# multimodallearning/DG-TTA

Measured on AMD Instinct MI355X. Metric: TTA-epochs/sec per GPU on 128^3 patch; Dice delta vs reference, higher is better.
Workload: dtype fp16

## Files before the change

### dg_tta_amd/_lib.py

```python
import ctypes as C
import os
from pathlib import Path

LIB_PATH = Path(__file__).resolve().parent / "libdgtta_hip.so"

_c_float_p = C.POINTER(C.c_float)
P, I, I64, F, SZ = C.c_void_p, C.c_int, C.c_int64, C.c_float, C.c_size_t

SIGNATURES = {
    "dgtta_version": (I, []),
    "dgtta_last_error": (C.c_char_p, []),
    "dgtta_reload_env": (I, []),
    "dgtta_mind3d_ws_bytes": (SZ, [I, I, I, I]),
    "dgtta_mind3d_fwd": (I, [P, P, F, I, C.POINTER(F), I, P, I, I, I, P, SZ, I, I, I, I, P]),
    "dgtta_gin_ws_bytes": (SZ, [I, I, I, I]),
    "dgtta_gin_chain_fwd": (I, [P, P, C.POINTER(I), C.POINTER(P), C.POINTER(P), P, P, SZ, I, I, I, I, P]),
    "dgtta_affine_warp3d_fwd": (I, [P, P, P, I, I, I, I, I, I, I, I, I, I, I, I, I, I, P, P]),
    "dgtta_affine_warp3d_bwd": (I, [P, P, P, I, I, I, I, I, I, I, I, I, I, I, I, I, P]),
    "dgtta_rf_field_ws_bytes": (SZ, [I, I, I, I]),
    "dgtta_rf_field_fwd": (I, [P, P, P, SZ, I, I, I, I, I, I, I, I, P]),
    "dgtta_diffeo_fields_ws_bytes": (SZ, [I, I, I, I]),
    "dgtta_diffeo_fields": (I, [P, F, P, P, P, SZ, I, I, I, I, I, P]),
    "dgtta_dense_warp3d_fwd": (I, [P, P, P, I, I, I, I, I, I, I, I, I, P]),
    "dgtta_dense_warp3d_bwd": (I, [P, P, P, I, I, I, I, I, I, I, I, I, P]),
    "dgtta_softdice_ws_bytes": (SZ, [I, I, I64]),
    "dgtta_softdice_fwd": (I, [P, P, P, P, P, SZ, I, I, I64, I, I, I, P]),
    "dgtta_softdice_bwd": (I, [P, P, P, P, P, F, P, I, I, I64, I, I, P]),
    "dgtta_softdice_bwd_t": (I, [P, P, P, P, P, F, P, I, I, I64, I, I, I, P]),
    "dgtta_softdice_probs_fwd": (I, [P, P, P, P, SZ, I, I, I64, I64, I64, I64, P]),
    "dgtta_softdice_probs_bwd": (I, [P, P, P, P, P, P, I, I, I64, I64, I64, I64, P]),
    "dgtta_dice_ce_ws_bytes": (SZ, [I, I, I64]),
    "dgtta_dice_ce_fwd": (I, [P, I, P, P, P, P, SZ, I, I, I64, F, I, P]),
    "dgtta_dice_ce_bwd": (I, [P, I, P, P, F, P, P, I, I, I, I64, P]),
    "dgtta_adamw_step": (I, [C.POINTER(P), C.POINTER(P), C.POINTER(P), C.POINTER(P), C.POINTER(I64), I, F, F, F, F, F,
                             I, F, P, P]),
    "dgtta_grads_nonfinite": (I, [C.POINTER(P), C.POINTER(I64), I, P, P]),
    "dgtta_conv3d_packed_bytes": (SZ, [I, I, I]),
    "dgtta_conv3d_pack_weights": (I, [P, P, I, I, I, I, I, P]),
    "dgtta_conv3d_stats_bytes": (SZ, [I, I, I, I, I]),
# ... 106 lines not shown
```

### dg_tta_amd/csrc/gin.hip

```cpp
#include "common.h"

namespace {

constexpr int TD = 8, TH = 8, TW = 32, HALO = 4, NT = 512;
constexpr int R0D = TD + 8, R0H = TH + 8, R0W = TW + 8;
constexpr int PW0 = 40, PW1 = 36, PW2 = 36, PW3 = 32;
constexpr int SZ_A = 2 * (TD + 4) * (TH + 4) * PW1 + 8;
constexpr int SZ_B = 2 * (TD + 6) * (TH + 6) * PW0 + 8;
constexpr int WTAB = 336;

struct GinArgs {
  const float *ker[4];
  const float *shift[4];
  int ksz[4];
};

__device__ __forceinline__ bool inside(int d, int h, int w, int D, int H, int W) {
  return (unsigned)d < (unsigned)D && (unsigned)h < (unsigned)H && (unsigned)w < (unsigned)W;
}

__global__ void gin_prep_kernel(GinArgs a, float *__restrict__ wtab) {
  const int b = blockIdx.x, tid = threadIdx.x;
  const int cin[4] = {1, 2, 2, 2}, cout[4] = {2, 2, 2, 1}, off[4] = {0, 54, 162, 270};
  float *wt = wtab + (int64_t)b * WTAB;
  for (int l = 0; l < 4; ++l) {
    const int k = a.ksz[l], rows = cout[l] * cin[l];
    for (int i = tid; i < rows * 27; i += blockDim.x) {
      const int r = i / 27, t = i % 27, co = r / cin[l], ci = r % cin[l];
      const float v = (k == 3) ? a.ker[l][((int64_t)b * rows + r) * 27 + t]
                               : ((t == 13) ? a.ker[l][(int64_t)b * rows + r] : 0.f);
      wt[off[l] + (ci * 27 + t) * cout[l] + co] = v;
    }
    if (tid < cout[l]) wt[324 + 2 * l + tid] = a.shift[l][b * cout[l] + tid];
  }
}

typedef __attribute__((ext_vector_type(2))) float f32x2_t;

__device__ __forceinline__ void pk_fma_blo(f32x2_t &acc, const f32x2_t &w, const f32x2_t &v) {
  asm volatile("v_pk_fma_f32 %0, %1, %2, %0 op_sel_hi:[1,0,1]" : "+v"(acc) : "v"(w), "v"(v));
}
__device__ __forceinline__ void pk_fma_bhi(f32x2_t &acc, const f32x2_t &w, const f32x2_t &v) {
  asm volatile("v_pk_fma_f32 %0, %1, %2, %0 op_sel:[0,1,0]" : "+v"(acc) : "v"(w), "v"(v));
}

template <int CIN, int COUT, bool ACT, int OD, int OH, int OW, int IPW, int OPW>
__device__ __forceinline__ void gin_layer(const float *sin, float *sout, const float *__restrict__ w ,
                                          const float *__restrict__ sh, int gd0, int gh0, int gw0, int D, int H, int W) {
  constexpr int ID = OD + 2, IH = OH + 2, NSX = (OW + 3) / 4, N = OD * OH * NSX;
  f32x2_t wreg[COUT == 2 ? CIN * 27 : 1];
  if (COUT == 2) {
#pragma unroll
    for (int i = 0; i < CIN * 27; ++i) wreg[i] = f32x2_t{w[2 * i], w[2 * i + 1]};
  }
  for (int s = threadIdx.x; s < N; s += NT) {
    const int xs = (s % NSX) * 4, y = (s / NSX) % OH, z = s / (NSX * OH);
    float o[COUT][4];
    if (COUT == 2) {
      f32x2_t acc[4];
#pragma unroll
      for (int j = 0; j < 4; ++j) acc[j] = f32x2_t{0.f, 0.f};
#pragma unroll
      for (int ci = 0; ci < CIN; ++ci)
#pragma unroll
        for (int kd = 0; kd < 3; ++kd)
#pragma unroll
          for (int kh = 0; kh < 3; ++kh) {
            const float *p = sin + ((ci * ID + z + kd) * IH + y + kh) * IPW + xs;
            const float4 q0 = *reinterpret_cast<const float4 *>(p);
            const float2 q1 = *reinterpret_cast<const float2 *>(p + 4);
            const f32x2_t vp[3] = {f32x2_t{q0.x, q0.y}, f32x2_t{q0.z, q0.w}, f32x2_t{q1.x, q1.y}};
#pragma unroll
            for (int kw = 0; kw < 3; ++kw) {
              const f32x2_t wv = wreg[ci * 27 + kd * 9 + kh * 3 + kw];
#pragma unroll
              for (int j = 0; j < 4; ++j) {
                if ((j + kw) & 1) pk_fma_bhi(acc[j], wv, vp[(j + kw) >> 1]);
                else pk_fma_blo(acc[j], wv, vp[(j + kw) >> 1]);
              }
            }
          }
#pragma unroll
      for (int j = 0; j < 4; ++j) {
        o[0][j] = acc[j][0];
        o[COUT - 1][j] = acc[j][1];
      }
    } else {
      float acc[4] = {0.f, 0.f, 0.f, 0.f};
#pragma unroll
      for (int ci = 0; ci < CIN; ++ci)
#pragma unroll
        for (int kd = 0; kd < 3; ++kd)
#pragma unroll
          for (int kh = 0; kh < 3; ++kh) {
            const float *p = sin + ((ci * ID + z + kd) * IH + y + kh) * IPW + xs;
            const float4 q0 = *reinterpret_cast<const float4 *>(p);
            const float2 q1 = *reinterpret_cast<const float2 *>(p + 4);
            const float v[6] = {q0.x, q0.y, q0.z, q0.w, q1.x, q1.y};
#pragma unroll
            for (int kw = 0; kw < 3; ++kw) {
              const float wv = w[ci * 27 + kd * 9 + kh * 3 + kw];
#pragma unroll
              for (int j = 0; j < 4; ++j) acc[j] = __builtin_fmaf(wv, v[j + kw], acc[j]);
            }
          }
#pragma unroll
      for (int j = 0; j < 4; ++j) o[0][j] = acc[j];
    }
    const bool zy_in = (unsigned)(gd0 + z) < (unsigned)D && (unsigned)(gh0 + y) < (unsigned)H;
#pragma unroll
    for (int co = 0; co < COUT; ++co) {
#pragma unroll
      for (int j = 0; j < 4; ++j) {
        const float v = o[co][j] + sh[co];
        const bool in = zy_in && (unsigned)(gw0 + xs + j) < (unsigned)W;
        o[co][j] = in ? (ACT ? lrelu(v, 0.01f) : v) : 0.f;
      }
      *reinterpret_cast<float4 *>(sout + ((co * OD + z) * OH + y) * OPW + xs) =
          make_float4(o[co][0], o[co][1], o[co][2], o[co][3]);
    }
  }
}

template <int CIN, int COUT, bool ACT, int OD, int OH, int OW, int IPW, int OPW>
__device__ __forceinline__ void gin_layer_k1(const float *sin, float *sout, const float *__restrict__ w,
                                             const float *__restrict__ sh, int gd0, int gh0, int gw0, int D, int H, int W) {
  constexpr int ID = OD + 2, IH = OH + 2, NSX = (OW + 3) / 4, N = OD * OH * NSX;
  float wc[COUT][CIN];
#pragma unroll
  for (int co = 0; co < COUT; ++co)
#pragma unroll
    for (int ci = 0; ci < CIN; ++ci) wc[co][ci] = w[(ci * 27 + 13) * COUT + co];
  for (int s = threadIdx.x; s < N; s += NT) {
    const int xs = (s % NSX) * 4, y = (s / NSX) % OH, z = s / (NSX * OH);
    float v[CIN][4];
#pragma unroll
    for (int ci = 0; ci < CIN; ++ci) {
      const float *p = sin + ((ci * ID + z + 1) * IH + y + 1) * IPW + xs + 1;
#pragma unroll
      for (int j = 0; j < 4; ++j) v[ci][j] = p[j];
    }
    const bool zy_in = (unsigned)(gd0 + z) < (unsigned)D && (unsigned)(gh0 + y) < (unsigned)H;
#pragma unroll
    for (int co = 0; co < COUT; ++co) {
      float o[4];
#pragma unroll
      for (int j = 0; j < 4; ++j) {
        float a = 0.f;
#pragma unroll
        for (int ci = 0; ci < CIN; ++ci) a = __builtin_fmaf(wc[co][ci], v[ci][j], a);
        a += sh[co];
        const bool in = zy_in && (unsigned)(gw0 + xs + j) < (unsigned)W;
        o[j] = in ? (ACT ? lrelu(a, 0.01f) : a) : 0.f;
      }
      *reinterpret_cast<float4 *>(sout + ((co * OD + z) * OH + y) * OPW + xs) = make_float4(o[0], o[1], o[2], o[3]);
    }
  }
}

__global__ __launch_bounds__(NT) void gin_chain_kernel(const float *__restrict__ x, const float *__restrict__ alpha,
                                                       const float *__restrict__ wtab, float *__restrict__ mixed,
                                                       double *__restrict__ partial, int D, int H, int W, int tilesD,
                                                       int tilesH, int tilesW, int ntiles, int k0, int k1, int k2,
                                                       int k3) {
  __shared__ __attribute__((aligned(16))) float bufA[SZ_A];
  __shared__ __attribute__((aligned(16))) float bufB[SZ_B];
  __shared__ float sred[16];
  constexpr int NPRE = R0D * R0H * R0W / NT;
  static_assert(R0D * R0H * R0W % NT == 0, "input tile must divide over the threads");

  const int tid = threadIdx.x;
  const int64_t V = (int64_t)D * H * W;
  const int per = tilesD * tilesH * tilesW;
  float pre[NPRE];
  auto fetch = [&](int tile) {
    const int b = tile / per, bid = tile % per;
    const int d0 = (bid / (tilesH * tilesW)) * TD, h0 = ((bid / tilesW) % tilesH) * TH, w0 = (bid % tilesW) * TW;
    const float *xb = x + (int64_t)b * V;
#pragma unroll
    for (int k = 0; k < NPRE; ++k) {
      const int i = tid + k * NT;
      const int iw = i % R0W, ih = (i / R0W) % R0H, id = i / (R0W * R0H);
      const int gd = d0 - HALO + id, gh = h0 - HALO + ih, gw = w0 - HALO + iw;
      const bool in = inside(gd, gh, gw, D, H, W);
      const float v = xb[in ? ((int64_t)gd * H + gh) * W + gw : 0];
      pre[k] = in ? v : 0.f;
    }
  };
  int tile = blockIdx.x;
  if (tile < ntiles) fetch(tile);
  for (; tile < ntiles; tile += gridDim.x) {
    const int b = tile / per, bid = tile % per;
    const int d0 = (bid / (tilesH * tilesW)) * TD, h0 = ((bid / tilesW) % tilesH) * TH, w0 = (bid % tilesW) * TW;
    const float *xb = x + (int64_t)b * V;
    const float *wt = wtab + (int64_t)b * WTAB;
#pragma unroll
    for (int k = 0; k < NPRE; ++k) bufA[tid + k * NT] = pre[k];
    __syncthreads();
    if (tile + (int)gridDim.x < ntiles) fetch(tile + gridDim.x);
    if (k0 == 1) gin_layer_k1<1, 2, true, TD + 6, TH + 6, TW + 6, R0W, PW0>(bufA, bufB, wt + 0, wt + 324, d0 - 3, h0 - 3, w0 - 3, D, H, W);
    else gin_layer<1, 2, true, TD + 6, TH + 6, TW + 6, R0W, PW0>(bufA, bufB, wt + 0, wt + 324, d0 - 3, h0 - 3, w0 - 3, D, H, W);
    __syncthreads();
    if (k1 == 1) gin_layer_k1<2, 2, true, TD + 4, TH + 4, TW + 4, PW0, PW1>(bufB, bufA, wt + 54, wt + 326, d0 - 2, h0 - 2, w0 - 2, D, H, W);
    else gin_layer<2, 2, true, TD + 4, TH + 4, TW + 4, PW0, PW1>(bufB, bufA, wt + 54, wt + 326, d0 - 2, h0 - 2, w0 - 2, D, H, W);
    __syncthreads();
    if (k2 == 1) gin_layer_k1<2, 2, true, TD + 2, TH + 2, TW + 2, PW1, PW2>(bufA, bufB, wt + 162, wt + 328, d0 - 1, h0 - 1, w0 - 1, D, H, W);
    else gin_layer<2, 2, true, TD + 2, TH + 2, TW + 2, PW1, PW2>(bufA, bufB, wt + 162, wt + 328, d0 - 1, h0 - 1, w0 - 1, D, H, W);
    __syncthreads();
    if (k3 == 1) gin_layer_k1<2, 1, false, TD, TH, TW, PW2, PW3>(bufB, bufA, wt + 270, wt + 330, d0, h0, w0, D, H, W);
    else gin_layer<2, 1, false, TD, TH, TW, PW2, PW3>(bufB, bufA, wt + 270, wt + 330, d0, h0, w0, D, H, W);
    __syncthreads();

    const float al = alpha[b];
    const float om = 1.0f - al;
    float s_in = 0.f, s_mx = 0.f;
    for (int i = tid; i < TD * TH * TW; i += NT) {
      int xw = i % TW, y = (i / TW) % TH, z = i / (TW * TH);
      int gd = d0 + z, gh = h0 + y, gw = w0 + xw;
      if (inside(gd, gh, gw, D, H, W)) {
        int64_t g = ((int64_t)gd * H + gh) * W + gw;
        float xi = xb[g];
        float t1 = al * bufA[i];
        float t2 = om * xi;
        float mx = t1 + t2;
        mixed[(int64_t)b * V + g] = mx;
        s_in += xi * xi;
        s_mx += mx * mx;
      }
    }
    float tin = block_sum(s_in, sred);
    float tmx = block_sum(s_mx, sred);
    if (tid == 0) {
      partial[((int64_t)b * per + bid) * 2 + 0] = (double)tin;
      partial[((int64_t)b * per + bid) * 2 + 1] = (double)tmx;
    }
    __syncthreads();
  }
}

__global__ void gin_norm_kernel(const double *__restrict__ partial, int per, float *__restrict__ norms) {
  __shared__ double sh[2][256];
  const int b = blockIdx.x;
  double s0 = 0.0, s1 = 0.0;
  for (int i = threadIdx.x; i < per; i += 256) {
    s0 += partial[((int64_t)b * per + i) * 2 + 0];
    s1 += partial[((int64_t)b * per + i) * 2 + 1];
  }
  sh[0][threadIdx.x] = s0;
  sh[1][threadIdx.x] = s1;
  __syncthreads();
  for (int o = 128; o > 0; o >>= 1) {
    if ((int)threadIdx.x < o) {
      sh[0][threadIdx.x] += sh[0][threadIdx.x + o];
      sh[1][threadIdx.x] += sh[1][threadIdx.x + o];
    }
    __syncthreads();
  }
  if (threadIdx.x == 0) {
    norms[2 * b + 0] = sqrtf((float)sh[0][0]);
    norms[2 * b + 1] = sqrtf((float)sh[1][0]);
  }
}

__global__ void gin_scale_kernel(float *__restrict__ out, const float *__restrict__ norms, int64_t V, int64_t total) {
  for (int64_t i = (int64_t)blockIdx.x * blockDim.x + threadIdx.x; i < total; i += (int64_t)gridDim.x * blockDim.x) {
    int64_t b = i / V;
    float r = 1.0f / (norms[2 * b + 1] + 1e-5f);
    out[i] = (out[i] * r) * norms[2 * b + 0];
  }
}

}

extern "C" size_t dgtta_gin_ws_bytes(int B, int D, int H, int W) {
  if (B <= 0 || D <= 0 || H <= 0 || W <= 0) return 0;
  size_t per = (size_t)cdiv(D, TD) * cdiv(H, TH) * cdiv(W, TW);
  return align_up((size_t)B * per * 2 * sizeof(double), 256) + align_up((size_t)B * 2 * sizeof(float), 256) +
         align_up((size_t)B * WTAB * sizeof(float), 256);
}

extern "C" int dgtta_gin_chain_fwd(const float *x, const float *alpha, const int *h_ksz, const float *const *h_ker,
                                   const float *const *h_shift, float *out, void *ws, size_t ws_bytes, int B, int D,
                                   int H, int W, void *stream) {
  DG_REQUIRE(x && alpha && h_ksz && h_ker && h_shift && out && ws, DGTTA_ERR_BADARG, "gin_chain_fwd: null pointer");
  DG_REQUIRE(B > 0 && D > 0 && H > 0 && W > 0, DGTTA_ERR_BADARG, "gin_chain_fwd: bad dims");
  DG_REQUIRE(ws_bytes >= dgtta_gin_ws_bytes(B, D, H, W), DGTTA_ERR_WORKSPACE, "gin_chain_fwd: workspace too small");
  GinArgs a;
  for (int l = 0; l < 4; ++l) {
    DG_REQUIRE(h_ksz[l] == 1 || h_ksz[l] == 3, DGTTA_ERR_UNSUPPORTED, "gin_chain_fwd: kernel size %d not in {1,3}",
               h_ksz[l]);
    DG_REQUIRE(h_ker[l] && h_shift[l], DGTTA_ERR_BADARG, "gin_chain_fwd: null layer pointer");
    a.ker[l] = h_ker[l];
    a.shift[l] = h_shift[l];
    a.ksz[l] = h_ksz[l];
  }
  hipStream_t st = (hipStream_t)stream;
  const int td = cdiv(D, TD), th = cdiv(H, TH), tw = cdiv(W, TW);
  DG_REQUIRE((int64_t)td * th * tw * B < (1ll << 31), DGTTA_ERR_UNSUPPORTED, "gin_chain_fwd: volume too large");
  const int per = td * th * tw;
  double *partial = (double *)ws;
  float *norms = (float *)((char *)ws + align_up((size_t)B * per * 2 * sizeof(double), 256));
  float *wtab = (float *)((char *)norms + align_up((size_t)B * 2 * sizeof(float), 256));
  const int64_t V = (int64_t)D * H * W;
  hipLaunchKernelGGL(gin_prep_kernel, dim3(B), dim3(128), 0, st, a, wtab);
  DG_CHECK_LAUNCH("gin_prep_kernel");
  const int ntiles = B * per;
  static const int ncu = [] {
    int dev = 0, n = 256;
    if (hipGetDevice(&dev) == hipSuccess) (void)hipDeviceGetAttribute(&n, hipDeviceAttributeMultiprocessorCount, dev);
    return n > 0 ? n : 256;
  }();
  hipLaunchKernelGGL(gin_chain_kernel, dim3(ntiles < ncu ? ntiles : ncu), dim3(NT), 0, st, x, alpha, wtab, out, partial, D,
                     H, W, td, th, tw, ntiles, a.ksz[0], a.ksz[1], a.ksz[2], a.ksz[3]);
  DG_CHECK_LAUNCH("gin_chain_kernel");
  hipLaunchKernelGGL(gin_norm_kernel, dim3(B), dim3(256), 0, st, partial, per, norms);
  DG_CHECK_LAUNCH("gin_norm_kernel");
  const int64_t total = (int64_t)B * V;
  int blocks = (int)((total + 255) / 256 < 4096 ? (total + 255) / 256 : 4096);
  hipLaunchKernelGGL(gin_scale_kernel, dim3(blocks), dim3(256), 0, st, out, norms, V, total);
  DG_CHECK_LAUNCH("gin_scale_kernel");
  return DGTTA_OK;
}
```

### dg_tta_amd/ops.py

```python
import ctypes as C

import torch

from . import _lib
from ._lib import check, ptr, require_cuda, stream_of

F32, BF16, F16 = 0, 1, 2


def dtype_code(torch_dtype):
    try:
        return {torch.float32: F32, torch.bfloat16: BF16, torch.float16: F16}[torch_dtype]
    except KeyError:
        raise ValueError(f"unsupported activation dtype {torch_dtype}") from None
PAD_ZEROS, PAD_BORDER = 0, 1
LINEAR, NEAREST = 0, 1


def _ws(nbytes, device):
    return torch.empty(max(int(nbytes), 256), dtype=torch.uint8, device=device)


def _f32c(t):
    return t.contiguous().float() if (t.dtype != torch.float32 or not t.is_contiguous()) else t
# ... 38 lines not shown
                                   ptr(out[sl]), int(ndhwc),
                                   int(out_ldc), dtype_code(out_dtype), ptr(ws), nbytes, bg, d, h, w,
                                   stream_of(img.device)), "dgtta_mind3d_fwd")
    return out


def gin_chain(x, alpha, ks, kers, shifts):
    require_cuda(x, alpha, *kers, *shifts)
    lib = _lib.load()
    b, c, d, h, w = x.shape
    assert c == 1 and len(ks) == len(kers) == len(shifts) == 4
    x = _f32c(x)
    alpha = _f32c(alpha)
    kers = [_f32c(k) for k in kers]
    shifts = [_f32c(s) for s in shifts]
    out = torch.empty_like(x)
    nbytes = lib.dgtta_gin_ws_bytes(b, d, h, w)
    ws = _ws(nbytes, x.device)
    ksz = (C.c_int * 4)(*[int(k) for k in ks])
    kp = (C.c_void_p * 4)(*[k.data_ptr() for k in kers])
    sp = (C.c_void_p * 4)(*[s.data_ptr() for s in shifts])
    check(lib.dgtta_gin_chain_fwd(ptr(x), ptr(alpha), ksz, kp, sp, ptr(out), ptr(ws), nbytes, b, d, h, w,
                                  stream_of(x.device)), "dgtta_gin_chain_fwd")
    return out


def _warp_layout(t):
    if is_cl3d(t) and t.shape[1] > 1:
        return t, 1, t.shape[1]
    t = t.contiguous()
    return t, 0, 0


def _warp_fwd_raw(src, theta, out_size, pad_mode, interp, algebra, sub_const):
    lib = _lib.load()
    b, c, ds, hs, wsz = src.shape
    dd, hd, wd = out_size
    src, ndhwc, ldc = _warp_layout(src)
    dst = empty_cl3d(b, c, dd, hd, wd, torch.float32, src.device) if ndhwc else \
        torch.empty((b, c, dd, hd, wd), dtype=torch.float32, device=src.device)
    check(lib.dgtta_affine_warp3d_fwd(ptr(src), ptr(theta), ptr(dst), b, c, ds, hs, wsz, dd, hd, wd, ndhwc, ldc, ldc,
                                      pad_mode, interp, int(algebra), ptr(sub_const), stream_of(src.device)),
          "dgtta_affine_warp3d_fwd")
    return dst


# ... 379 lines not shown
```

### include/dgtta.h

```cpp
#ifndef DGTTA_H
#define DGTTA_H

#include <stddef.h>
#include <stdint.h>

#ifdef __cplusplus
extern "C" {
#endif

#define DGTTA_OK 0
#define DGTTA_ERR_BADARG (-1)
#define DGTTA_ERR_UNSUPPORTED (-2)
#define DGTTA_ERR_WORKSPACE (-3)
#define DGTTA_ERR_LAUNCH (-4)

#define DGTTA_F32 0
#define DGTTA_BF16 1
#define DGTTA_F16 2

#define DGTTA_PAD_ZEROS 0
#define DGTTA_PAD_BORDER 1
#define DGTTA_INTERP_LINEAR 0
#define DGTTA_INTERP_NEAREST 1

int dgtta_version(void);
const char *dgtta_last_error(void);
int dgtta_reload_env(void);

size_t dgtta_mind3d_ws_bytes(int B, int D, int H, int W);
int dgtta_mind3d_fwd(const float *img, const float *noise, float randn_weighting, int delta, const float *h_taps,
                     int ntaps, void *out, int out_ndhwc, int out_ldc, int out_dtype, void *ws, size_t ws_bytes, int B,
                     int D, int H, int W, void *stream);

size_t dgtta_gin_ws_bytes(int B, int D, int H, int W);
int dgtta_gin_chain_fwd(const float *x, const float *alpha, const int *h_ksz, const float *const *h_ker,
                        const float *const *h_shift, float *out, void *ws, size_t ws_bytes, int B, int D, int H,
                        int W, void *stream);

int dgtta_affine_warp3d_fwd(const float *src, const float *theta, float *dst, int B, int C, int Ds, int Hs,
                            int Ws, int Dd, int Hd, int Wd, int ndhwc, int src_ldc, int dst_ldc, int pad_mode,
                            int interp_mode, int tta_grid_algebra, const float *sub_const_dev, void *stream);
int dgtta_affine_warp3d_bwd(const float *grad_dst, const float *theta, float *grad_src, int B, int C, int Ds,
                            int Hs, int Ws, int Dd, int Hd, int Wd, int ndhwc, int src_ldc, int dst_ldc,
                            int pad_mode, int tta_grid_algebra, void *stream);

size_t dgtta_rf_field_ws_bytes(int P, int Dl, int Hl, int Wl);
int dgtta_rf_field_fwd(const float *draw, float *field, void *ws, size_t ws_bytes, int P, int k, int Dl, int Hl, int Wl,
                       int D, int H, int W, void *stream);
size_t dgtta_diffeo_fields_ws_bytes(int N, int D, int H, int W);
int dgtta_diffeo_fields(const float *field, float factor, float *disp, float *inverse, void *ws, size_t ws_bytes, int N,
                        int D, int H, int W, int time_steps, void *stream);
int dgtta_dense_warp3d_fwd(const float *src, const float *disp, float *dst, int B, int C, int D, int H, int W, int ndhwc,
                           int src_ldc, int dst_ldc, int pad_mode, void *stream);
int dgtta_dense_warp3d_bwd(const float *grad_dst, const float *disp, float *grad_src, int B, int C, int D, int H, int W,
                           int ndhwc, int src_ldc, int dst_ldc, int pad_mode, void *stream);

size_t dgtta_softdice_ws_bytes(int B, int C, int64_t V);
int dgtta_softdice_fwd(const float *la, const float *lb, float *dice, float *loss, void *ws, size_t ws_bytes,
                       int B, int C, int64_t V, int ldc, int start_class, int guard_items, void *stream);
int dgtta_softdice_bwd(const float *la, const float *lb, float *grad_la, float *grad_lb, const void *ws,
// ... 164 lines not shown
```

Baseline: 6.529.

## Restructure GIN chain kernel as depth-marching ring-buffered layer pipeline

Replaces the 3D-tile GIN conv chain, which recomputed halos across all four layers in a shared-memory cube, with a kernel that marches along depth over an H×W column. Each layer runs in its own thread role and keeps only a four-plane ring buffer in shared memory, and thread roles stay a fixed number of planes apart, separated by barriers. Weights are held in registers per role, and the depth range is split into segments to fill the CUs. The aim is to cut redundant halo recomputation and shared-memory footprint. It also adds a per-sample GIN weight entry point and batched weight prep. The cost is a larger block, a barrier on every plane step, and more complex partial-sum indexing.

```diff
diff --git a/dg_tta_amd/_lib.py b/dg_tta_amd/_lib.py
--- a/dg_tta_amd/_lib.py
+++ b/dg_tta_amd/_lib.py
@@ -15,6 +15,7 @@
     "dgtta_mind3d_fwd": (I, [P, P, F, I, C.POINTER(F), I, P, I, I, I, P, SZ, I, I, I, I, P]),
     "dgtta_gin_ws_bytes": (SZ, [I, I, I, I]),
     "dgtta_gin_chain_fwd": (I, [P, P, C.POINTER(I), C.POINTER(P), C.POINTER(P), P, P, SZ, I, I, I, I, P]),
+    "dgtta_gin_chain_fwd_per_sample": (I, [P, P, C.POINTER(I), C.POINTER(P), C.POINTER(P), P, P, SZ, I, I, I, I, P]),
     "dgtta_affine_warp3d_fwd": (I, [P, P, P, I, I, I, I, I, I, I, I, I, I, I, I, I, I, P, P]),
     "dgtta_affine_warp3d_bwd": (I, [P, P, P, I, I, I, I, I, I, I, I, I, I, I, I, I, P]),
     "dgtta_rf_field_ws_bytes": (SZ, [I, I, I, I]),
diff --git a/dg_tta_amd/csrc/gin.hip b/dg_tta_amd/csrc/gin.hip
--- a/dg_tta_amd/csrc/gin.hip
+++ b/dg_tta_amd/csrc/gin.hip
@@ -1,37 +1,38 @@
 #include "common.h"
 
+#include <vector>
+
 namespace {
 
-constexpr int TD = 8, TH = 8, TW = 32, HALO = 4, NT = 512;
-constexpr int R0D = TD + 8, R0H = TH + 8, R0W = TW + 8;
-constexpr int PW0 = 40, PW1 = 36, PW2 = 36, PW3 = 32;
-constexpr int SZ_A = 2 * (TD + 4) * (TH + 4) * PW1 + 8;
-constexpr int SZ_B = 2 * (TD + 6) * (TH + 6) * PW0 + 8;
+constexpr int CH = 16, CW = 32, NTM = 768, RING = 4, DBLK = 8;
+constexpr int INH = CH + 8, INPW = 40, IN_SZ = INH * INPW;
+constexpr int H0 = CH + 6, PW0 = 40, SZ0 = 2 * H0 * PW0;
+constexpr int H1 = CH + 4, PW1 = 36, SZ1 = 2 * H1 * PW1;
+constexpr int H2 = CH + 2, PW2 = 36, SZ2 = 2 * H2 * PW2;
 constexpr int WTAB = 336;
 
+constexpr int PREP_B = 8;
 struct GinArgs {
-  const float *ker[4];
-  const float *shift[4];
-  int ksz[4];
+  const float *ker[PREP_B][4];
+  const float *shift[PREP_B][4];
+  int ksz[PREP_B][4];
+  int b0;
 };
 
-__device__ __forceinline__ bool inside(int d, int h, int w, int D, int H, int W) {
-  return (unsigned)d < (unsigned)D && (unsigned)h < (unsigned)H && (unsigned)w < (unsigned)W;
-}
-
 __global__ void gin_prep_kernel(GinArgs a, float *__restrict__ wtab) {
-  const int b = blockIdx.x, tid = threadIdx.x;
+  const int i = blockIdx.x, tid = threadIdx.x;
   const int cin[4] = {1, 2, 2, 2}, cout[4] = {2, 2, 2, 1}, off[4] = {0, 54, 162, 270};
-  float *wt = wtab + (int64_t)b * WTAB;
+  float *wt = wtab + (int64_t)(a.b0 + i) * WTAB;
   for (int l = 0; l < 4; ++l) {
-    const int k = a.ksz[l], rows = cout[l] * cin[l];
-    for (int i = tid; i < rows * 27; i += blockDim.x) {
-      const int r = i / 27, t = i % 27, co = r / cin[l], ci = r % cin[l];
-      const float v = (k == 3) ? a.ker[l][((int64_t)b * rows + r) * 27 + t]
-                               : ((t == 13) ? a.ker[l][(int64_t)b * rows + r] : 0.f);
+    const int k = a.ksz[i][l], rows = cout[l] * cin[l];
+    const float *ker = a.ker[i][l];
+    for (int e = tid; e < rows * 27; e += blockDim.x) {
+      const int r = e / 27, t = e % 27, co = r / cin[l], ci = r % cin[l];
+      const float v = (k == 3) ? ker[r * 27 + t] : ((t == 13) ? ker[r] : 0.f);
       wt[off[l] + (ci * 27 + t) * cout[l] + co] = v;
     }
-    if (tid < cout[l]) wt[324 + 2 * l + tid] = a.shift[l][b * cout[l] + tid];
+    if (tid < cout[l]) wt[324 + 2 * l + tid] = a.shift[i][l][tid];
+    if (tid == 0) wt[332 + l] = (float)k;
   }
 }
 
@@ -44,197 +45,283 @@
   asm volatile("v_pk_fma_f32 %0, %1, %2, %0 op_sel:[0,1,0]" : "+v"(acc) : "v"(w), "v"(v));
 }
 
-template <int CIN, int COUT, bool ACT, int OD, int OH, int OW, int IPW, int OPW>
-__device__ __forceinline__ void gin_layer(const float *sin, float *sout, const float *__restrict__ w ,
-                                          const float *__restrict__ sh, int gd0, int gh0, int gw0, int D, int H, int W) {
-  constexpr int ID = OD + 2, IH = OH + 2, NSX = (OW + 3) / 4, N = OD * OH * NSX;
-  f32x2_t wreg[COUT == 2 ? CIN * 27 : 1];
-  if (COUT == 2) {
-#pragma unroll
-    for (int i = 0; i < CIN * 27; ++i) wreg[i] = f32x2_t{w[2 * i], w[2 * i + 1]};
-  }
-  for (int s = threadIdx.x; s < N; s += NT) {
-    const int xs = (s % NSX) * 4, y = (s / NSX) % OH, z = s / (NSX * OH);
-    float o[COUT][4];
-    if (COUT == 2) {
-      f32x2_t acc[4];
-#pragma unroll
-      for (int j = 0; j < 4; ++j) acc[j] = f32x2_t{0.f, 0.f};
-#pragma unroll
-      for (int ci = 0; ci < CIN; ++ci)
-#pragma unroll
-        for (int kd = 0; kd < 3; ++kd)
-#pragma unroll
-          for (int kh = 0; kh < 3; ++kh) {
-            const float *p = sin + ((ci * ID + z + kd) * IH + y + kh) * IPW + xs;
-            const float4 q0 = *reinterpret_cast<const float4 *>(p);
-            const float2 q1 = *reinterpret_cast<const float2 *>(p + 4);
-            const f32x2_t vp[3] = {f32x2_t{q0.x, q0.y}, f32x2_t{q0.z, q0.w}, f32x2_t{q1.x, q1.y}};
-#pragma unroll
-            for (int kw = 0; kw < 3; ++kw) {
-              const f32x2_t wv = wreg[ci * 27 + kd * 9 + kh * 3 + kw];
-#pragma unroll
-              for (int j = 0; j < 4; ++j) {
-                if ((j + kw) & 1) pk_fma_bhi(acc[j], wv, vp[(j + kw) >> 1]);
-                else pk_fma_blo(acc[j], wv, vp[(j + kw) >> 1]);
-              }
+template <int CIN, int COUT, bool K1>
+struct LayerW {
+  f32x2_t pk[(!K1 && COUT == 2) ? CIN * 27 : 1];
+  float sc[(!K1 && COUT == 1) ? CIN * 27 : 1];
+  float c1[COUT][CIN];
+  float sh[COUT];
+  __device__ __forceinline__ void load(const float *__restrict__ w, const float *__restrict__ shp) {
+    if constexpr (K1) {
+#pragma unroll
+      for (int co = 0; co < COUT; ++co)
+#pragma unroll
+        for (int ci = 0; ci < CIN; ++ci) c1[co][ci] = w[(ci * 27 + 13) * COUT + co];
+    } else if constexpr (COUT == 2) {
+#pragma unroll
+      for (int i = 0; i < CIN * 27; ++i) {
+        pk[i] = f32x2_t{w[2 * i], w[2 * i + 1]};
+        asm volatile("" : "+v"(pk[i]));
+      }
+    } else {
+#pragma unroll
+      for (int i = 0; i < CIN * 27; ++i) sc[i] = w[i];
+    }
+#pragma unroll
+    for (int co = 0; co < COUT; ++co) sh[co] = shp[co];
+  }
+};
+
+template <int CIN, int COUT, bool K1, int IH, int IPW>
+__device__ __forceinline__ void gin_strip(const float *const (&pl)[3], const LayerW<CIN, COUT, K1> &lw, int y, int xs,
+                                          float (&o)[COUT][4]) {
+  if constexpr (K1) {
+    float v[CIN][4];
+#pragma unroll
+    for (int ci = 0; ci < CIN; ++ci) {
+      const float *p = pl[1] + (ci * IH + y + 1) * IPW + xs + 1;
+#pragma unroll
+      for (int j = 0; j < 4; ++j) v[ci][j] = p[j];
+    }
+#pragma unroll
+    for (int co = 0; co < COUT; ++co)
+#pragma unroll
+      for (int j = 0; j < 4; ++j) {
+        float a = 0.f;
+#pragma unroll
+        for (int ci = 0; ci < CIN; ++ci) a = __builtin_fmaf(lw.c1[co][ci], v[ci][j], a);
+        o[co][j] = a;
+      }
+  } else if constexpr (COUT == 2) {
+    f32x2_t acc[4];
+#pragma unroll
+    for (int j = 0; j < 4; ++j) acc[j] = f32x2_t{0.f, 0.f};
+#pragma unroll
+    for (int ci = 0; ci < CIN; ++ci)
+#pragma unroll
+      for (int kd = 0; kd < 3; ++kd)
+#pragma unroll
+        for (int kh = 0; kh < 3; ++kh) {
+          const float *p = pl[kd] + (ci * IH + y + kh) * IPW + xs;
+          const float4 q0 = *reinterpret_cast<const float4 *>(p);
+          const float2 q1 = *reinterpret_cast<const float2 *>(p + 4);
+          const f32x2_t vp[3] = {f32x2_t{q0.x, q0.y}, f32x2_t{q0.z, q0.w}, f32x2_t{q1.x, q1.y}};
+#pragma unroll
+          for (int kw = 0; kw < 3; ++kw) {
+            const f32x2_t wv = lw.pk[ci * 27 + kd * 9 + kh * 3 + kw];
+#pragma unroll
+            for (int j = 0; j < 4; ++j) {
+              if ((j + kw) & 1) pk_fma_bhi(acc[j], wv, vp[(j + kw) >> 1]);
+              else pk_fma_blo(acc[j], wv, vp[(j + kw) >> 1]);
             }
           }
-#pragma unroll
-      for (int j = 0; j < 4; ++j) {
-        o[0][j] = acc[j][0];
-        o[COUT - 1][j] = acc[j][1];
+        }
+#pragma unroll
+    for (int j = 0; j < 4; ++j) {
+      o[0][j] = acc[j][0];
+      o[COUT - 1][j] = acc[j][1];
+    }
+  } else {
+    float acc[4] = {0.f, 0.f, 0.f, 0.f};
+#pragma unroll
+    for (int ci = 0; ci < CIN; ++ci)
+#pragma unroll
+      for (int kd = 0; kd < 3; ++kd)
+#pragma unroll
+        for (int kh = 0; kh < 3; ++kh) {
+          const float *p = pl[kd] + (ci * IH + y + kh) * IPW + xs;
+          const float4 q0 = *reinterpret_cast<const float4 *>(p);
+          const float2 q1 = *reinterpret_cast<const float2 *>(p + 4);
+          const float v[6] = {q0.x, q0.y, q0.z, q0.w, q1.x, q1.y};
+#pragma unroll
+          for (int kw = 0; kw < 3; ++kw) {
+            const float wv = lw.sc[ci * 27 + kd * 9 + kh * 3 + kw];
+#pragma unroll
+            for (int j = 0; j < 4; ++j) acc[j] = __builtin_fmaf(wv, v[j + kw], acc[j]);
+          }
+        }
+#pragma unroll
+    for (int j = 0; j < 4; ++j) o[0][j] = acc[j];
+  }
+}
+
+__device__ __forceinline__ int ring_slot(int p) { return (p + 8) & (RING - 1); }
+
+template <int CIN, bool K1, int IH, int IPW, int ISZ, int OH, int OPW>
+__device__ __forceinline__ void gin_plane_strip(const float *rin, float *po, const LayerW<CIN, 2, K1> &lw, int p, int y,
+                                                int xs, int gh, int gw0, int D, int H, int W) {
+  float o[2][4];
+  const bool row_in = (unsigned)p < (unsigned)D && (unsigned)gh < (unsigned)H;
+  if ((unsigned)p < (unsigned)D) {
+    const float *const pl[3] = {rin + ring_slot(p - 1) * ISZ, rin + ring_slot(p) * ISZ, rin + ring_slot(p + 1) * ISZ};
+    gin_strip<CIN, 2, K1, IH, IPW>(pl, lw, y, xs, o);
+  } else {
+#pragma unroll
+    for (int j = 0; j < 4; ++j) o[0][j] = o[1][j] = 0.f;
+  }
+#pragma unroll
+  for (int co = 0; co < 2; ++co) {
+#pragma unroll
+    for (int j = 0; j < 4; ++j) {
+      const float v = o[co][j] + lw.sh[co];
+      const bool in = row_in && (unsigned)(gw0 + xs + j) < (unsigned)W;
+      o[co][j] = in ? lrelu(v, 0.01f) : 0.f;
+    }
+    *reinterpret_cast<float4 *>(po + (co * OH + y) * OPW + xs) = make_float4(o[co][0], o[co][1], o[co][2], o[co][3]);
+  }
+}
+
+struct March {
+  const float *xb;
+  const float *wt;
+  int ds, de, nsteps;
+  int h0, w0, D, H, W;
+};
+
+template <bool K1>
+__device__ __forceinline__ void gin_role_l0(const March &m, float *sIn, float *sA0, int lt) {
+  LayerW<1, 2, K1> lw;
+  lw.load(m.wt + 0, m.wt + 324);
+  constexpr int NSX = PW0 / 4;
+  const bool task = lt < H0 * NSX, ftask = lt < INH * (INPW / 4);
+  const int y = task ? lt / NSX : 0, xs = (lt % NSX) * 4;
+  const int fr = ftask ? lt / (INPW / 4) : 0, fc = (lt % (INPW / 4)) * 4;
+  const int gh_f = m.h0 - 4 + fr, gw_f = m.w0 - 4 + fc;
+  const bool vec_ok = (m.W & 3) == 0 && (reinterpret_cast<uintptr_t>(m.xb) & 15) == 0;
+  auto fetch = [&](int p, float (&r)[4]) {
+#pragma unroll
+    for (int j = 0; j < 4; ++j) r[j] = 0.f;
+    if (ftask && (unsigned)p < (unsigned)m.D && (unsigned)gh_f < (unsigned)m.H) {
+      const float *row = m.xb + ((int64_t)p * m.H + gh_f) * m.W;
+      if (vec_ok && gw_f >= 0 && gw_f + 3 < m.W) {
+        const float4 q = *reinterpret_cast<const float4 *>(row + gw_f);
+        r[0] = q.x, r[1] = q.y, r[2] = q.z, r[3] = q.w;
+      } else {
+#pragma unroll
+        for (int j = 0; j < 4; ++j)
+          if ((unsigned)(gw_f + j) < (unsigned)m.W) r[j] = row[gw_f + j];
       }
-    } else {
-      float acc[4] = {0.f, 0.f, 0.f, 0.f};
-#pragma unroll
-      for (int ci = 0; ci < CIN; ++ci)
-#pragma unroll
-        for (int kd = 0; kd < 3; ++kd)
-#pragma unroll
-          for (int kh = 0; kh < 3; ++kh) {
-            const float *p = sin + ((ci * ID + z + kd) * IH + y + kh) * IPW + xs;
-            const float4 q0 = *reinterpret_cast<const float4 *>(p);
-            const float2 q1 = *reinterpret_cast<const float2 *>(p + 4);
-            const float v[6] = {q0.x, q0.y, q0.z, q0.w, q1.x, q1.y};
-#pragma unroll
-            for (int kw = 0; kw < 3; ++kw) {
-              const float wv = w[ci * 27 + kd * 9 + kh * 3 + kw];
-#pragma unroll
-              for (int j = 0; j < 4; ++j) acc[j] = __builtin_fmaf(wv, v[j + kw], acc[j]);
-            }
-          }
-#pragma unroll
-      for (int j = 0; j < 4; ++j) o[0][j] = acc[j];
-    }
-    const bool zy_in = (unsigned)(gd0 + z) < (unsigned)D && (unsigned)(gh0 + y) < (unsigned)H;
-#pragma unroll
-    for (int co = 0; co < COUT; ++co) {
-#pragma unroll
-      for (int j = 0; j < 4; ++j) {
-        const float v = o[co][j] + sh[co];
-        const bool in = zy_in && (unsigned)(gw0 + xs + j) < (unsigned)W;
-        o[co][j] = in ? (ACT ? lrelu(v, 0.01f) : v) : 0.f;
+    }
+  };
+  auto stash = [&](int p, const float (&r)[4]) {
+    if (ftask)
+      *reinterpret_cast<float4 *>(sIn + ring_slot(p) * IN_SZ + fr * INPW + fc) = make_float4(r[0], r[1], r[2], r[3]);
+  };
+  for (int q = 0; q < 3; ++q) {
+    float r[4];
+    fetch(m.ds - 4 + q, r);
+    stash(m.ds - 4 + q, r);
+  }
+  __syncthreads();
+  for (int s = 0; s < m.nsteps; ++s) {
+    const int p = m.ds - 3 + s;
+    const bool fneed = p + 2 < m.de + 4;
+    float r[4];
+    if (fneed) fetch(p + 2, r);
+    if (task && p < m.de + 3)
+      gin_plane_strip<1, K1, INH, INPW, IN_SZ, H0, PW0>(sIn, sA0 + ring_slot(p) * SZ0, lw, p, y, xs, m.h0 - 3 + y,
+                                                       m.w0 - 3, m.D, m.H, m.W);
+    if (fneed) stash(p + 2, r);
+    __syncthreads();
+  }
+}
+
+template <bool K1, int OFF, int LAG, int IH, int IPW, int ISZ, int OH, int OPW, int OSZ>
+__device__ __forceinline__ void gin_role_mid(const March &m, const float *rin, float *rout, const float *w,
+                                             const float *sh, int lt) {
+  LayerW<2, 2, K1> lw;
+  lw.load(w, sh);
+  constexpr int NSX = OPW / 4;
+  const bool task = lt < OH * NSX;
+  const int y = task ? lt / NSX : 0, xs = (lt % NSX) * 4;
+  __syncthreads();
+  for (int s = 0; s < m.nsteps; ++s) {
+    const int p = m.ds - 3 + s - LAG;
+    if (task && p >= m.ds - OFF && p < m.de + OFF)
+      gin_plane_strip<2, K1, IH, IPW, ISZ, OH, OPW>(rin, rout + ring_slot(p) * OSZ, lw, p, y, xs, m.h0 - OFF + y,
+                                                   m.w0 - OFF, m.D, m.H, m.W);
+    __syncthreads();
+  }
+}
+
+template <bool K1>
+__device__ __forceinline__ void gin_role_l3(const March &m, const float *sA2, float al, float *__restrict__ mixed_b,
+                                            double *__restrict__ part , int lt) {
+  LayerW<2, 1, K1> lw;
+  lw.load(m.wt + 270, m.wt + 330);
+  const int y = lt / (CW / 4), xs = (lt % (CW / 4)) * 4, gh = m.h0 + y, gw = m.w0 + xs;
+  const float om = 1.0f - al;
+  float s_in = 0.f, s_mx = 0.f;
+  __syncthreads();
+  for (int s = 0; s < m.nsteps; ++s) {
+    const int p = m.ds - 9 + s;
+    if (p >= m.ds && p < m.de) {
+      const int64_t g = ((int64_t)p * m.H + gh) * m.W + gw;
+      float xi[4];
+#pragma unroll
+      for (int j = 0; j < 4; ++j) xi[j] = (gh < m.H && gw + j < m.W) ? m.xb[g + j] : 0.f;
+      const float *const pl[3] = {sA2 + ring_slot(p - 1) * SZ2, sA2 + ring_slot(p) * SZ2, sA2 + ring_slot(p + 1) * SZ2};
+      float o[1][4];
+      gin_strip<2, 1, K1, H2, PW2>(pl, lw, y, xs, o);
+#pragma unroll
+      for (int j = 0; j < 4; ++j)
+        if (gh < m.H && gw + j < m.W) {
+          const float res = o[0][j] + lw.sh[0];
+          float t1 = al * res;
+          float t2 = om * xi[j];
+          float mx = t1 + t2;
+          mixed_b[g + j] = mx;
+          s_in += xi[j] * xi[j];
+          s_mx += mx * mx;
+        }
+      if ((p & (DBLK - 1)) == DBLK - 1 || p == m.de - 1) {
+        const float tin = wave_sum(s_in), tmx = wave_sum(s_mx);
+        if ((lt & 63) == 0) {
+          double *q = part + ((p / DBLK) * 2 + (lt >> 6)) * 2;
+          q[0] = (double)tin;
+          q[1] = (double)tmx;
+        }
+        s_in = s_mx = 0.f;
       }
-      *reinterpret_cast<float4 *>(sout + ((co * OD + z) * OH + y) * OPW + xs) =
-          make_float4(o[co][0], o[co][1], o[co][2], o[co][3]);
-    }
-  }
-}
-
-template <int CIN, int COUT, bool ACT, int OD, int OH, int OW, int IPW, int OPW>
-__device__ __forceinline__ void gin_layer_k1(const float *sin, float *sout, const float *__restrict__ w,
-                                             const float *__restrict__ sh, int gd0, int gh0, int gw0, int D, int H, int W) {
-  constexpr int ID = OD + 2, IH = OH + 2, NSX = (OW + 3) / 4, N = OD * OH * NSX;
-  float wc[COUT][CIN];
-#pragma unroll
-  for (int co = 0; co < COUT; ++co)
-#pragma unroll
-    for (int ci = 0; ci < CIN; ++ci) wc[co][ci] = w[(ci * 27 + 13) * COUT + co];
-  for (int s = threadIdx.x; s < N; s += NT) {
-    const int xs = (s % NSX) * 4, y = (s / NSX) % OH, z = s / (NSX * OH);
-    float v[CIN][4];
-#pragma unroll
-    for (int ci = 0; ci < CIN; ++ci) {
-      const float *p = sin + ((ci * ID + z + 1) * IH + y + 1) * IPW + xs + 1;
-#pragma unroll
-      for (int j = 0; j < 4; ++j) v[ci][j] = p[j];
-    }
-    const bool zy_in = (unsigned)(gd0 + z) < (unsigned)D && (unsigned)(gh0 + y) < (unsigned)H;
-#pragma unroll
-    for (int co = 0; co < COUT; ++co) {
-      float o[4];
-#pragma unroll
-      for (int j = 0; j < 4; ++j) {
-        float a = 0.f;
-#pragma unroll
-        for (int ci = 0; ci < CIN; ++ci) a = __builtin_fmaf(wc[co][ci], v[ci][j], a);
-        a += sh[co];
-        const bool in = zy_in && (unsigned)(gw0 + xs + j) < (unsigned)W;
-        o[j] = in ? (ACT ? lrelu(a, 0.01f) : a) : 0.f;
-      }
-      *reinterpret_cast<float4 *>(sout + ((co * OD + z) * OH + y) * OPW + xs) = make_float4(o[0], o[1], o[2], o[3]);
-    }
-  }
-}
-
-__global__ __launch_bounds__(NT) void gin_chain_kernel(const float *__restrict__ x, const float *__restrict__ alpha,
-                                                       const float *__restrict__ wtab, float *__restrict__ mixed,
-                                                       double *__restrict__ partial, int D, int H, int W, int tilesD,
-                                                       int tilesH, int tilesW, int ntiles, int k0, int k1, int k2,
-                                                       int k3) {
-  __shared__ __attribute__((aligned(16))) float bufA[SZ_A];
-  __shared__ __attribute__((aligned(16))) float bufB[SZ_B];
-  __shared__ float sred[16];
-  constexpr int NPRE = R0D * R0H * R0W / NT;
-  static_assert(R0D * R0H * R0W % NT == 0, "input tile must divide over the threads");
-
-  const int tid = threadIdx.x;
+    }
+    __syncthreads();
+  }
+}
+
+__global__ __launch_bounds__(NTM) void gin_chain_kernel(const float *__restrict__ x, const float *__restrict__ alpha,
+                                                        const float *__restrict__ wtab, float *__restrict__ mixed,
+                                                        double *__restrict__ partial, int D, int H, int W, int colsW,
+                                                        int ncols, int nblk, int bps, int nseg) {
+  __shared__ __attribute__((aligned(16))) float sIn[RING * IN_SZ + 8];
+  __shared__ __attribute__((aligned(16))) float sA0[RING * SZ0 + 8];
+  __shared__ __attribute__((aligned(16))) float sA1[RING * SZ1 + 8];
+  __shared__ __attribute__((aligned(16))) float sA2[RING * SZ2 + 8];
+
+  const int tid = threadIdx.x, wave = __builtin_amdgcn_readfirstlane(tid >> 6);
+  const int item = blockIdx.x, seg = item % nseg, col = (item / nseg) % ncols, b = item / (nseg * ncols);
   const int64_t V = (int64_t)D * H * W;
-  const int per = tilesD * tilesH * tilesW;
-  float pre[NPRE];
-  auto fetch = [&](int tile) {
-    const int b = tile / per, bid = tile % per;
-    const int d0 = (bid / (tilesH * tilesW)) * TD, h0 = ((bid / tilesW) % tilesH) * TH, w0 = (bid % tilesW) * TW;
-    const float *xb = x + (int64_t)b * V;
-#pragma unroll
-    for (int k = 0; k < NPRE; ++k) {
-      const int i = tid + k * NT;
-      const int iw = i % R0W, ih = (i / R0W) % R0H, id = i / (R0W * R0H);
-      const int gd = d0 - HALO + id, gh = h0 - HALO + ih, gw = w0 - HALO + iw;
-      const bool in = inside(gd, gh, gw, D, H, W);
-      const float v = xb[in ? ((int64_t)gd * H + gh) * W + gw : 0];
-      pre[k] = in ? v : 0.f;
-    }
-  };
-  int tile = blockIdx.x;
-  if (tile < ntiles) fetch(tile);
-  for (; tile < ntiles; tile += gridDim.x) {
-    const int b = tile / per, bid = tile % per;
-    const int d0 = (bid / (tilesH * tilesW)) * TD, h0 = ((bid / tilesW) % tilesH) * TH, w0 = (bid % tilesW) * TW;
-    const float *xb = x + (int64_t)b * V;
-    const float *wt = wtab + (int64_t)b * WTAB;
-#pragma unroll
-    for (int k = 0; k < NPRE; ++k) bufA[tid + k * NT] = pre[k];
-    __syncthreads();
-    if (tile + (int)gridDim.x < ntiles) fetch(tile + gridDim.x);
-    if (k0 == 1) gin_layer_k1<1, 2, true, TD + 6, TH + 6, TW + 6, R0W, PW0>(bufA, bufB, wt + 0, wt + 324, d0 - 3, h0 - 3, w0 - 3, D, H, W);
-    else gin_layer<1, 2, true, TD + 6, TH + 6, TW + 6, R0W, PW0>(bufA, bufB, wt + 0, wt + 324, d0 - 3, h0 - 3, w0 - 3, D, H, W);
-    __syncthreads();
-    if (k1 == 1) gin_layer_k1<2, 2, true, TD + 4, TH + 4, TW + 4, PW0, PW1>(bufB, bufA, wt + 54, wt + 326, d0 - 2, h0 - 2, w0 - 2, D, H, W);
-    else gin_layer<2, 2, true, TD + 4, TH + 4, TW + 4, PW0, PW1>(bufB, bufA, wt + 54, wt + 326, d0 - 2, h0 - 2, w0 - 2, D, H, W);
-    __syncthreads();
-    if (k2 == 1) gin_layer_k1<2, 2, true, TD + 2, TH + 2, TW + 2, PW1, PW2>(bufA, bufB, wt + 162, wt + 328, d0 - 1, h0 - 1, w0 - 1, D, H, W);
-    else gin_layer<2, 2, true, TD + 2, TH + 2, TW + 2, PW1, PW2>(bufA, bufB, wt + 162, wt + 328, d0 - 1, h0 - 1, w0 - 1, D, H, W);
-    __syncthreads();
-    if (k3 == 1) gin_layer_k1<2, 1, false, TD, TH, TW, PW2, PW3>(bufB, bufA, wt + 270, wt + 330, d0, h0, w0, D, H, W);
-    else gin_layer<2, 1, false, TD, TH, TW, PW2, PW3>(bufB, bufA, wt + 270, wt + 330, d0, h0, w0, D, H, W);
-    __syncthreads();
-
-    const float al = alpha[b];
-    const float om = 1.0f - al;
-    float s_in = 0.f, s_mx = 0.f;
-    for (int i = tid; i < TD * TH * TW; i += NT) {
-      int xw = i % TW, y = (i / TW) % TH, z = i / (TW * TH);
-      int gd = d0 + z, gh = h0 + y, gw = w0 + xw;
-      if (inside(gd, gh, gw, D, H, W)) {
-        int64_t g = ((int64_t)gd * H + gh) * W + gw;
-        float xi = xb[g];
-        float t1 = al * bufA[i];
-        float t2 = om * xi;
-        float mx = t1 + t2;
-        mixed[(int64_t)b * V + g] = mx;
-        s_in += xi * xi;
-        s_mx += mx * mx;
-      }
-    }
-    float tin = block_sum(s_in, sred);
-    float tmx = block_sum(s_mx, sred);
-    if (tid == 0) {
-      partial[((int64_t)b * per + bid) * 2 + 0] = (double)tin;
-      partial[((int64_t)b * per + bid) * 2 + 1] = (double)tmx;
-    }
-    __syncthreads();
+  March m;
+  m.xb = x + (int64_t)b * V;
+  m.wt = wtab + (int64_t)b * WTAB;
+  m.ds = seg * bps * DBLK;
+  m.de = min(D, m.ds + bps * DBLK);
+  m.nsteps = m.de - m.ds + 9;
+  m.h0 = (col / colsW) * CH, m.w0 = (col % colsW) * CW, m.D = D, m.H = H, m.W = W;
+  const bool k1[4] = {m.wt[332] == 1.f, m.wt[333] == 1.f, m.wt[334] == 1.f, m.wt[335] == 1.f};
+
+  if (wave < 4) {
+    if (k1[0]) gin_role_l0<true>(m, sIn, sA0, tid);
+    else gin_role_l0<false>(m, sIn, sA0, tid);
+  } else if (wave < 7) {
+    if (k1[1]) gin_role_mid<true, 2, 2, H0, PW0, SZ0, H1, PW1, SZ1>(m, sA0, sA1, m.wt + 54, m.wt + 326, tid - 256);
+    else gin_role_mid<false, 2, 2, H0, PW0, SZ0, H1, PW1, SZ1>(m, sA0, sA1, m.wt + 54, m.wt + 326, tid - 256);
+  } else if (wave < 10) {
+    if (k1[2]) gin_role_mid<true, 1, 4, H1, PW1, SZ1, H2, PW2, SZ2>(m, sA1, sA2, m.wt + 162, m.wt + 328, tid - 448);
+    else gin_role_mid<false, 1, 4, H1, PW1, SZ1, H2, PW2, SZ2>(m, sA1, sA2, m.wt + 162, m.wt + 328, tid - 448);
+  } else {
+    double *part = partial + ((int64_t)(b * ncols + col) * nblk) * 4;
+    if (k1[3]) gin_role_l3<true>(m, sA2, alpha[b], mixed + (int64_t)b * V, part, tid - 640);
+    else gin_role_l3<false>(m, sA2, alpha[b], mixed + (int64_t)b * V, part, tid - 640);
   }
 }
 
@@ -272,46 +359,55 @@
 
 }
 
+static size_t gin_partials(int D, int H, int W) { return (size_t)cdiv(H, CH) * cdiv(W, CW) * cdiv(D, DBLK) * 2; }
+
 extern "C" size_t dgtta_gin_ws_bytes(int B, int D, int H, int W) {
   if (B <= 0 || D <= 0 || H <= 0 || W <= 0) return 0;
-  size_t per = (size_t)cdiv(D, TD) * cdiv(H, TH) * cdiv(W, TW);
+  size_t per = gin_partials(D, H, W);
   return align_up((size_t)B * per * 2 * sizeof(double), 256) + align_up((size_t)B * 2 * sizeof(float), 256) +
          align_up((size_t)B * WTAB * sizeof(float), 256);
 }
 
-extern "C" int dgtta_gin_chain_fwd(const float *x, const float *alpha, const int *h_ksz, const float *const *h_ker,
-                                   const float *const *h_shift, float *out, void *ws, size_t ws_bytes, int B, int D,
-                                   int H, int W, void *stream) {
-  DG_REQUIRE(x && alpha && h_ksz && h_ker && h_shift && out && ws, DGTTA_ERR_BADARG, "gin_chain_fwd: null pointer");
+static int gin_chain_launch(const float *x, const float *alpha, const int *h_ksz, const float *const *h_ker,
+                            const float *const *h_shift, float *out, void *ws, size_t ws_bytes, int B, int D, int H, int W,
+                            void *stream) {
   DG_REQUIRE(B > 0 && D > 0 && H > 0 && W > 0, DGTTA_ERR_BADARG, "gin_chain_fwd: bad dims");
   DG_REQUIRE(ws_bytes >= dgtta_gin_ws_bytes(B, D, H, W), DGTTA_ERR_WORKSPACE, "gin_chain_fwd: workspace too small");
-  GinArgs a;
-  for (int l = 0; l < 4; ++l) {
-    DG_REQUIRE(h_ksz[l] == 1 || h_ksz[l] == 3, DGTTA_ERR_UNSUPPORTED, "gin_chain_fwd: kernel size %d not in {1,3}",
-               h_ksz[l]);
-    DG_REQUIRE(h_ker[l] && h_shift[l], DGTTA_ERR_BADARG, "gin_chain_fwd: null layer pointer");
-    a.ker[l] = h_ker[l];
-    a.shift[l] = h_shift[l];
-    a.ksz[l] = h_ksz[l];
+  for (int i = 0; i < 4 * B; ++i) {
+    DG_REQUIRE(h_ksz[i] == 1 || h_ksz[i] == 3, DGTTA_ERR_UNSUPPORTED, "gin_chain_fwd: kernel size %d not in {1,3}",
+               h_ksz[i]);
+    DG_REQUIRE(h_ker[i] && h_shift[i], DGTTA_ERR_BADARG, "gin_chain_fwd: null layer pointer");
   }
   hipStream_t st = (hipStream_t)stream;
-  const int td = cdiv(D, TD), th = cdiv(H, TH), tw = cdiv(W, TW);
-  DG_REQUIRE((int64_t)td * th * tw * B < (1ll << 31), DGTTA_ERR_UNSUPPORTED, "gin_chain_fwd: volume too large");
-  const int per = td * th * tw;
+  const int colsW = cdiv(W, CW), ncols = cdiv(H, CH) * colsW, nblk = cdiv(D, DBLK);
+  const int64_t V = (int64_t)D * H * W;
+  DG_REQUIRE((int64_t)ncols * nblk * B < (1ll << 29) && V + 4 < (1ll << 31), DGTTA_ERR_UNSUPPORTED,
+             "gin_chain_fwd: volume too large");
+  const int per = (int)gin_partials(D, H, W);
   double *partial = (double *)ws;
   float *norms = (float *)((char *)ws + align_up((size_t)B * per * 2 * sizeof(double), 256));
   float *wtab = (float *)((char *)norms + align_up((size_t)B * 2 * sizeof(float), 256));
-  const int64_t V = (int64_t)D * H * W;
-  hipLaunchKernelGGL(gin_prep_kernel, dim3(B), dim3(128), 0, st, a, wtab);
-  DG_CHECK_LAUNCH("gin_prep_kernel");
-  const int ntiles = B * per;
+  for (int b0 = 0; b0 < B; b0 += PREP_B) {
+    GinArgs a;
+    const int n = B - b0 < PREP_B ? B - b0 : PREP_B;
+    for (int i = 0; i < PREP_B; ++i)
+      for (int l = 0; l < 4; ++l) {
+        const int j = (b0 + (i < n ? i : 0)) * 4 + l;
+        a.ker[i][l] = h_ker[j], a.shift[i][l] = h_shift[j], a.ksz[i][l] = h_ksz[j];
+      }
+    a.b0 = b0;
+    hipLaunchKernelGGL(gin_prep_kernel, dim3(n), dim3(128), 0, st, a, wtab);
+    DG_CHECK_LAUNCH("gin_prep_kernel");
+  }
   static const int ncu = [] {
     int dev = 0, n = 256;
     if (hipGetDevice(&dev) == hipSuccess) (void)hipDeviceGetAttribute(&n, hipDeviceAttributeMultiprocessorCount, dev);
     return n > 0 ? n : 256;
   }();
-  hipLaunchKernelGGL(gin_chain_kernel, dim3(ntiles < ncu ? ntiles : ncu), dim3(NT), 0, st, x, alpha, wtab, out, partial, D,
-                     H, W, td, th, tw, ntiles, a.ksz[0], a.ksz[1], a.ksz[2], a.ksz[3]);
+  const int want = cdiv(ncu, ncols * B), most = nblk / 2 > 1 ? nblk / 2 : 1;
+  const int bps = cdiv(nblk, want < most ? want : most), nseg = cdiv(nblk, bps);
+  hipLaunchKernelGGL(gin_chain_kernel, dim3(B * ncols * nseg), dim3(NTM), 0, st, x, alpha, wtab, out, partial, D, H, W,
+                     colsW, ncols, nblk, bps, nseg);
   DG_CHECK_LAUNCH("gin_chain_kernel");
   hipLaunchKernelGGL(gin_norm_kernel, dim3(B), dim3(256), 0, st, partial, per, norms);
   DG_CHECK_LAUNCH("gin_norm_kernel");
@@ -321,3 +417,33 @@
   DG_CHECK_LAUNCH("gin_scale_kernel");
   return DGTTA_OK;
 }
+
+extern "C" int dgtta_gin_chain_fwd(const float *x, const float *alpha, const int *h_ksz, const float *const *h_ker,
+                                   const float *const *h_shift, float *out, void *ws, size_t ws_bytes, int B, int D,
+                                   int H, int W, void *stream) {
+  DG_REQUIRE(x && alpha && h_ksz && h_ker && h_shift && out && ws, DGTTA_ERR_BADARG, "gin_chain_fwd: null pointer");
+  DG_REQUIRE(B > 0 && B < (1 << 24), DGTTA_ERR_BADARG, "gin_chain_fwd: bad dims");
+  const int cin[4] = {1, 2, 2, 2}, cout[4] = {2, 2, 2, 1};
+  std::vector<int> ksz(4 * (size_t)B);
+  std::vector<const float *> ker(4 * (size_t)B), shift(4 * (size_t)B);
+  for (int l = 0; l < 4; ++l) {
+    DG_REQUIRE(h_ksz[l] == 1 || h_ksz[l] == 3, DGTTA_ERR_UNSUPPORTED, "gin_chain_fwd: kernel size %d not in {1,3}",
+               h_ksz[l]);
+    DG_REQUIRE(h_ker[l] && h_shift[l], DGTTA_ERR_BADARG, "gin_chain_fwd: null layer pointer");
+    const int64_t taps = h_ksz[l] == 3 ? 27 : 1;
+    for (int b = 0; b < B; ++b) {
+      ksz[4 * b + l] = h_ksz[l];
+      ker[4 * b + l] = h_ker[l] + (int64_t)b * cout[l] * cin[l] * taps;
+      shift[4 * b + l] = h_shift[l] + (int64_t)b * cout[l];
+    }
+  }
+  return gin_chain_launch(x, alpha, ksz.data(), ker.data(), shift.data(), out, ws, ws_bytes, B, D, H, W, stream);
+}
+
+extern "C" int dgtta_gin_chain_fwd_per_sample(const float *x, const float *alpha, const int *h_ksz,
+                                              const float *const *h_ker, const float *const *h_shift, float *out, void *ws,
+                                              size_t ws_bytes, int B, int D, int H, int W, void *stream) {
+  DG_REQUIRE(x && alpha && h_ksz && h_ker && h_shift && out && ws, DGTTA_ERR_BADARG, "gin_chain_fwd_per_sample: null pointer");
+  DG_REQUIRE(B > 0 && B < (1 << 24), DGTTA_ERR_BADARG, "gin_chain_fwd_per_sample: bad dims");
+  return gin_chain_launch(x, alpha, h_ksz, h_ker, h_shift, out, ws, ws_bytes, B, D, H, W, stream);
+}
diff --git a/dg_tta_amd/ops.py b/dg_tta_amd/ops.py
--- a/dg_tta_amd/ops.py
+++ b/dg_tta_amd/ops.py
@@ -84,6 +84,27 @@
     sp = (C.c_void_p * 4)(*[s.data_ptr() for s in shifts])
     check(lib.dgtta_gin_chain_fwd(ptr(x), ptr(alpha), ksz, kp, sp, ptr(out), ptr(ws), nbytes, b, d, h, w,
                                   stream_of(x.device)), "dgtta_gin_chain_fwd")
+    return out
+
+
+def gin_chain_per_sample(x, alpha, draws):
+    b, c, d, h, w = x.shape
+    assert c == 1 and len(draws) == b and alpha.numel() == b
+    lib = _lib.load()
+    x, alpha = _f32c(x), _f32c(alpha)
+    ksz, keep = [], []
+    for ks, kers, shifts in draws:
+        assert len(ks) == len(kers) == len(shifts) == 4
+        require_cuda(x, alpha, *kers, *shifts)
+        ksz += [int(k) for k in ks]
+        keep += [(_f32c(k), _f32c(s)) for k, s in zip(kers, shifts)]
+    out = torch.empty_like(x)
+    nbytes = lib.dgtta_gin_ws_bytes(b, d, h, w)
+    ws = _ws(nbytes, x.device)
+    check(lib.dgtta_gin_chain_fwd_per_sample(ptr(x), ptr(alpha), (C.c_int * (4 * b))(*ksz),
+                                             (C.c_void_p * (4 * b))(*[k.data_ptr() for k, _ in keep]),
+                                             (C.c_void_p * (4 * b))(*[s.data_ptr() for _, s in keep]), ptr(out), ptr(ws),
+                                             nbytes, b, d, h, w, stream_of(x.device)), "dgtta_gin_chain_fwd_per_sample")
     return out
 
 
diff --git a/include/dgtta.h b/include/dgtta.h
--- a/include/dgtta.h
+++ b/include/dgtta.h
@@ -36,6 +36,9 @@
 int dgtta_gin_chain_fwd(const float *x, const float *alpha, const int *h_ksz, const float *const *h_ker,
                         const float *const *h_shift, float *out, void *ws, size_t ws_bytes, int B, int D, int H,
                         int W, void *stream);
+int dgtta_gin_chain_fwd_per_sample(const float *x, const float *alpha, const int *h_ksz, const float *const *h_ker,
+                                   const float *const *h_shift, float *out, void *ws, size_t ws_bytes, int B, int D,
+                                   int H, int W, void *stream);
 
 int dgtta_affine_warp3d_fwd(const float *src, const float *theta, float *dst, int B, int C, int Ds, int Hs,
                             int Ws, int Dd, int Hd, int Wd, int ndhwc, int src_ldc, int dst_ldc, int pad_mode,
```

After: 6.506, median of 5. No clear change (-0.4%).
